# PKU-EPIC/HOTrack

Hardware: AMD Instinct MI355X
Metric: HandTrackNet point-cloud frames/sec (N=1024) (higher is better)
Workload: dtype f32; 1 GPU; HandTrackNet forward, batch=64 synthetic 1024-pt clouds per GPU (BASELINE configs[1]); per_gpu_batch=64, global_batch=64, npoints=1024, parallelism=dp1 (independent batches, no collective), world_size=1, resident_batches_rotated=5, dead_attention_elided=True, fused_sa_kernels=True, launch=hipGraph replay, batches_in_flight=4, hip_hw_queues=4, sa_compute_units=256, weights=deterministic random init (no checkpoint available offline)

## Files before the change

hotrack_amd/csrc/capi.hip:

```cpp
#include <stdlib.h>

#include "pn2_common.h"
#include "../../include/pn2_ext.h"

namespace pn2 {
static thread_local int g_last_hip_error = 0;
void set_last_hip_error(int e) { g_last_hip_error = e; }

int fps_dispatch(int b, int n, int m, const float *xyz, float *temp, int *idx, hipStream_t st, int force_threads,
                 const int *skip_flags, int nflags, float *radii);
int fps_tie_check(int b, int n, int m, int m1, const float *xyz, const int *idx, const float *radii, int *flags, hipStream_t st);
bool fps_knn_supported(int n, int nq, int k);
bool ball_tie_supported(long b, long n, long m, long m2);
int ball_tie_dispatch(int b, int n, int m, float radius, int nsample, const float *xyz, int *idx, const int *picks, float *new_xyz_out,
                      float *new_xyz_copy, int copy_ld, int m2, const float *radii, int *flags, hipStream_t st, int *counts);
bool three_nn_interp_supported(long b, long n, long m, long c, long ldp, long ldo);
int three_nn_interp_dispatch(int b, int n, int m, int c, const float *unknown, const float *known, const float *points, int ldp,
                             float *out, int ldo, hipStream_t st);
int fps_knn_dispatch(int b, int n, int m, const float *xyz, int *idx, float *radii, int nq, int k, int k2, const float *query,
                     int *kidx, int *kidx2, hipStream_t st);
int ball_query_dispatch(int b, int n, int m, float radius, int nsample, const float *new_xyz, const float *xyz,
                        int *idx, hipStream_t st, const int *picks, float *new_xyz_out, float *new_xyz_copy, int copy_ld, int *counts);
int three_nn_dispatch(int b, int n, int m, const float *unknown, const float *known, float *dist2, int *idx,
                      hipStream_t st, bool weights);
int interp_pm_dispatch(int b, int c, int m, int n, const float *points, int ldp, const int *idx, const float *weight,
                       float *out, int ldo, hipStream_t st);
int knn_dispatch(int b, int n, int m, int k, const float *unknown, const float *known, float *dist2, int *idx,
                 hipStream_t st, int k2, int *idx2);
int group_fwd_dispatch(int b, int c, int n, int npoints, int nsample, const float *points, const int *idx,
                       float *out, hipStream_t st);
int group_bwd_dispatch(int b, int c, int n, int npoints, int nsample, const float *grad_out, const int *idx,
                       float *grad_points, hipStream_t st);
int interp_fwd_dispatch(int b, int c, int m, int n, const float *points, const int *idx, const float *weight,
                        float *out, hipStream_t st);
int interp_bwd_dispatch(int b, int c, int n, int m, const float *grad_out, const int *idx, const float *weight,
                        float *grad_points, hipStream_t st);
}

using namespace pn2;

#define PN2_REQ(cond, code) \
// ... 206 lines not shown

int pn2x_three_nn_weights(int b, int n, int m, const float *unknown, const float *known, float *weight, int *idx,
                          void *stream) {
    PN2_REQ(b >= 0 && n >= 0 && m >= 3, PN2_EINVAL);
    if (b == 0 || n == 0) return PN2_OK;
    PN2_REQ(unknown && known && weight && idx, PN2_ENULL);
    PN2_REQ(b <= 65535 && fits_int((long)n * 3) && fits_int((long)m * 3), PN2_ERANGE);
    return three_nn_dispatch(b, n, m, unknown, known, weight, idx, (hipStream_t)stream, true);
}

int pn2x_three_nn_interpolate_pm_supported(int b, int n, int m, int c, int ldp, int ldo) {
    return three_nn_interp_supported(b, n, m, c, ldp, ldo) ? 1 : 0;
}

int pn2x_three_nn_interpolate_pm(int b, int n, int m, int c, const float *unknown, const float *known, const float *points, int ldp,
                                 float *out, int ldo, void *stream) {
    PN2_REQ(b >= 0 && n >= 0 && m >= 3 && c >= 1 && ldp >= c && ldo >= c, PN2_EINVAL);
    if (b == 0 || n == 0) return PN2_OK;
    PN2_REQ(unknown && known && points && out, PN2_ENULL);
    PN2_REQ(b <= 65535 && fits_int((long)n * 3) && fits_int((long)m * 3), PN2_ERANGE);
    return three_nn_interp_dispatch(b, n, m, c, unknown, known, points, ldp, out, ldo, (hipStream_t)stream);
}

int pn2x_three_interpolate_pm(int b, int c, int m, int n, const float *points, int ldp, const int *idx,
                              const float *weight, float *out, int ldo, void *stream) {
    PN2_REQ(b >= 0 && c >= 0 && m >= 1 && n >= 0 && ldp >= c && ldo >= c, PN2_EINVAL);
    if (b == 0 || c == 0 || n == 0) return PN2_OK;
    PN2_REQ(points && idx && weight && out, PN2_ENULL);
    PN2_REQ(fits_int((long)n * 3), PN2_ERANGE);
    return interp_pm_dispatch(b, c, m, n, points, ldp, idx, weight, out, ldo, (hipStream_t)stream);
}

}
```

hotrack_amd/csrc/nn_search.hip:

```cpp
#include "pn2_common.h"
#include "knn_wave.h"

namespace pn2 {

constexpr int kNnTile = 2048;

template <int THREADS, bool WEIGHTS>
__global__ void __launch_bounds__(THREADS)
three_nn_kernel(int n, int m, const float *__restrict__ unknown_all, const float *__restrict__ known_all,
                float *__restrict__ dist2_all, int *__restrict__ idx_all) {
    extern __shared__ __attribute__((aligned(16))) float4 sk[];
    const int b = blockIdx.y;
    const float *__restrict__ known = known_all + (size_t)b * m * 3;
    const int q = blockIdx.x * THREADS + threadIdx.x;
    const bool active = q < n;
    const float *__restrict__ u = unknown_all + ((size_t)b * n + (active ? q : 0)) * 3;
    const float ux = u[0], uy = u[1], uz = u[2];

    float b1 = __builtin_inff(), b2 = __builtin_inff(), b3 = __builtin_inff();
    int i1 = 0, i2 = 0, i3 = 0;

    for (int t0 = 0; t0 < m; t0 += kNnTile) {
        const int tn = (m - t0) < kNnTile ? (m - t0) : kNnTile;
        if (t0 > 0) __syncthreads();
// ... 70 lines not shown
    if (c > 0) {
        sd[c - 1][0][ql] = b1; sd[c - 1][1][ql] = b2; sd[c - 1][2][ql] = b3;
        si[c - 1][0][ql] = i1; si[c - 1][1][ql] = i2; si[c - 1][2][ql] = i3;
    }
    __syncthreads();
    if (c != 0 || !active) return;
#pragma unroll
    for (int cc = 0; cc < 3; ++cc)
#pragma unroll
        for (int e = 0; e < 3; ++e) insert(sd[cc][e][ql], si[cc][e][ql]);
    float *od = dist2_all + ((size_t)b * n + q) * 3;
    int *oi = idx_all + ((size_t)b * n + q) * 3;
    if constexpr (WEIGHTS) {
        const float r1 = 1.0f / (__builtin_sqrtf(b1) + 1e-8f), r2 = 1.0f / (__builtin_sqrtf(b2) + 1e-8f),
                    r3 = 1.0f / (__builtin_sqrtf(b3) + 1e-8f);
        const float norm = (r1 + r2) + r3;
        od[0] = r1 / norm; od[1] = r2 / norm; od[2] = r3 / norm;
    } else {
        od[0] = b1; od[1] = b2; od[2] = b3;
    }
    oi[0] = i1; oi[1] = i2; oi[2] = i3;
}

__global__ void __launch_bounds__(256)
three_nn_interp_kernel(int n, int m, int c4, const float *__restrict__ unknown_all, const float *__restrict__ known_all,
                       const float *__restrict__ points_all, int ldp, float *__restrict__ out_all, int ldo) {
    extern __shared__ __attribute__((aligned(16))) float4 sk[];
    __shared__ float sd[3][3][64];
    __shared__ int si[3][3][64];
    __shared__ float fw[3][64];
    __shared__ int fi[3][64];
    const int b = blockIdx.y;
    const float *__restrict__ known = known_all + (size_t)b * m * 3;
    const int ql = threadIdx.x & 63, c = threadIdx.x >> 6;
    const int q = blockIdx.x * 64 + ql;
    const bool active = q < n;
    const float *__restrict__ u = unknown_all + ((size_t)b * n + (active ? q : 0)) * 3;
    const float ux = u[0], uy = u[1], uz = u[2];
    for (int p = threadIdx.x; p < m; p += 256) {
        const float *src = known + (size_t)3 * p;
        sk[p] = make_float4(src[0], src[1], src[2], 0.f);
    }
    __syncthreads();
    float b1 = __builtin_inff(), b2 = __builtin_inff(), b3 = __builtin_inff();
    int i1 = 0, i2 = 0, i3 = 0;
    auto insert = [&](float d, int k) {
        const bool lt1 = d < b1, lt2 = d < b2, lt3 = d < b3;
        b3 = lt2 ? b2 : (lt3 ? d : b3);
        i3 = lt2 ? i2 : (lt3 ? k : i3);
        b2 = lt1 ? b1 : (lt2 ? d : b2);
        i2 = lt1 ? i1 : (lt2 ? k : i2);
        b1 = lt1 ? d : b1;
        i1 = lt1 ? k : i1;
    };
    const int len = (m + 3) / 4, p0 = c * len, p1 = min(m, p0 + len);
#pragma unroll 4
    for (int p = p0; p < p1; ++p) {
        const float4 kp = sk[p];
        insert(sqdist(ux, uy, uz, kp.x, kp.y, kp.z), p);
    }
    if (c > 0) {
        sd[c - 1][0][ql] = b1; sd[c - 1][1][ql] = b2; sd[c - 1][2][ql] = b3;
        si[c - 1][0][ql] = i1; si[c - 1][1][ql] = i2; si[c - 1][2][ql] = i3;
    }
    __syncthreads();
    if (c == 0) {
#pragma unroll
        for (int cc = 0; cc < 3; ++cc)
#pragma unroll
            for (int e = 0; e < 3; ++e) insert(sd[cc][e][ql], si[cc][e][ql]);
        const float r1 = 1.0f / (__builtin_sqrtf(b1) + 1e-8f), r2 = 1.0f / (__builtin_sqrtf(b2) + 1e-8f),
                    r3 = 1.0f / (__builtin_sqrtf(b3) + 1e-8f);
        const float norm = (r1 + r2) + r3;
        fw[0][ql] = r1 / norm; fw[1][ql] = r2 / norm; fw[2][ql] = r3 / norm;
        fi[0][ql] = i1; fi[1][ql] = i2; fi[2][ql] = i3;
    }
    __syncthreads();
    const int rows = min(64, n - (int)blockIdx.x * 64);
    const float *__restrict__ src = points_all + (size_t)b * m * ldp;
    float *__restrict__ dst = out_all + ((size_t)b * n + (size_t)blockIdx.x * 64) * ldo;
    for (int e = threadIdx.x; e < rows * c4; e += 256) {
        const int r = e / c4, col = e - r * c4;
        const float w0 = fw[0][r], w1 = fw[1][r], w2 = fw[2][r];
        const float4 a0 = *reinterpret_cast<const float4 *>(src + (size_t)fi[0][r] * ldp + 4 * col);
        const float4 a1 = *reinterpret_cast<const float4 *>(src + (size_t)fi[1][r] * ldp + 4 * col);
        const float4 a2 = *reinterpret_cast<const float4 *>(src + (size_t)fi[2][r] * ldp + 4 * col);
        float4 o;
        o.x = __builtin_fmaf(w2, a2.x, __builtin_fmaf(w0, a0.x, w1 * a1.x));
        o.y = __builtin_fmaf(w2, a2.y, __builtin_fmaf(w0, a0.y, w1 * a1.y));
        o.z = __builtin_fmaf(w2, a2.z, __builtin_fmaf(w0, a0.z, w1 * a1.z));
        o.w = __builtin_fmaf(w2, a2.w, __builtin_fmaf(w0, a0.w, w1 * a1.w));
        *reinterpret_cast<float4 *>(dst + (size_t)r * ldo + 4 * col) = o;
    }
}

bool three_nn_interp_supported(long b, long n, long m, long c, long ldp, long ldo) {
    return b * n >= 16384 && b * n < 256L * 1024 && m >= 16 && m <= kNnTile && c >= 4 && c % 4 == 0 && ldp % 4 == 0 && ldo % 4 == 0;
}

int three_nn_interp_dispatch(int b, int n, int m, int c, const float *unknown, const float *known, const float *points, int ldp,
                             float *out, int ldo, hipStream_t st) {
    if (b == 0 || n == 0) return PN2_OK;
    if (!three_nn_interp_supported(b, n, m, c, ldp, ldo) || (((uintptr_t)points | (uintptr_t)out) % 16) != 0) return PN2_ERANGE;
    dim3 grid((n + 63) / 64, b);
    hipLaunchKernelGGL(three_nn_interp_kernel, grid, dim3(256), (size_t)m * sizeof(float4), st, n, m, c / 4, unknown, known, points, ldp, out, ldo);
    return check_launch();
}

int three_nn_dispatch(int b, int n, int m, const float *unknown, const float *known, float *dist2,
                      int *idx, hipStream_t st, bool weights) {
    if (b == 0 || n == 0) return PN2_OK;
    if ((long)b * n < 256L * 1024 && m >= 16 && m <= kNnTile) {
        dim3 grid((n + 63) / 64, b);
        const size_t lds_split = (size_t)m * sizeof(float4);
        if (weights) hipLaunchKernelGGL((three_nn_split_kernel<true>), grid, dim3(256), lds_split, st, n, m, unknown, known, dist2, idx);
        else hipLaunchKernelGGL((three_nn_split_kernel<false>), grid, dim3(256), lds_split, st, n, m, unknown, known, dist2, idx);
        return check_launch();
    }
    const int tile_cap = m < kNnTile ? m : kNnTile;
    const size_t lds = (size_t)(tile_cap > 0 ? tile_cap : 1) * sizeof(float4);
    if ((long)b * n < 256L * 1024) {
        dim3 grid((n + 63) / 64, b);
        if (weights) hipLaunchKernelGGL((three_nn_kernel<64, true>), grid, dim3(64), lds, st, n, m, unknown, known, dist2, idx);
        else hipLaunchKernelGGL((three_nn_kernel<64, false>), grid, dim3(64), lds, st, n, m, unknown, known, dist2, idx);
    } else {
        dim3 grid((n + 255) / 256, b);
        if (weights) hipLaunchKernelGGL((three_nn_kernel<256, true>), grid, dim3(256), lds, st, n, m, unknown, known, dist2, idx);
        else hipLaunchKernelGGL((three_nn_kernel<256, false>), grid, dim3(256), lds, st, n, m, unknown, known, dist2, idx);
// ... 91 lines not shown
```

hotrack_amd/csrc/sa_fused.hip:

```cpp
#include <stdlib.h>

#include "pn2_common.h"
#include "../../include/pn2_ext.h"

#ifndef SA_PAD
#define SA_PAD 4
#endif

#ifndef SA_DEFER_EPILOGUE
#define SA_DEFER_EPILOGUE 0
#endif
#ifndef SA_OVERLAP_WRITEOUT
#define SA_OVERLAP_WRITEOUT 1
#endif
#ifndef SA_SCALAR_L1
#define SA_SCALAR_L1 0
#endif
#ifndef SA_LOADER_PRIO
#define SA_LOADER_PRIO 0
#endif
#ifndef SA_PROBE
#define SA_PROBE 0
#endif
#ifndef SA_PREFETCH
// ... 815 lines not shown
    switch (a.K) {
        case 16: return launch_sa_k<C1, C2, C3, WC, RTC, MINW, NB1, 16>(b, a, st);
        case 32: return launch_sa_k<C1, C2, C3, WC, RTC, MINW, NB1, 32>(b, a, st);
        case 64: return launch_sa_k<C1, C2, C3, WC, RTC, MINW, NB1, 64>(b, a, st);
    }
    return PN2_ERANGE;
}

#ifndef SA_RTC128
#define SA_RTC128 2
#endif
#ifndef SA_NB1
#define SA_NB1 2
#endif
static long long *g_sa_trace = nullptr;
static bool sa_ranges_ok(long b, long n, long s, long k, long a1f_ld, long cadd_ld, long c3, long out_s, long out_c) {
    const long lim = 0xffffffffL;
    if (out_s < 0 || out_c < 0 || 4 * ((s - 1) * out_s + (c3 - 1) * out_c + 1) >= lim) return false;
    return n < (1L << 24) && s < (1L << 24) && 4 * a1f_ld < (1L << 24) && 4 * cadd_ld < (1L << 24) &&
           4 * b * n * (a1f_ld > 3 ? a1f_ld : 3) <= lim && 4 * s * (cadd_ld > 3 ? cadd_ld : 3) <= lim && 4 * s * k <= lim;
}

constexpr int kClsThreads = 1024;
__global__ __launch_bounds__(kClsThreads) void sa_class_lists_kernel(int M, int S, int N, const int *__restrict__ counts,
                                                                      int *__restrict__ list, int *__restrict__ sizes) {
    __shared__ int scan[3][kClsThreads];
    const int tid = (int)threadIdx.x;
    const int per = (M + kClsThreads - 1) / kClsThreads;
    const long lo = (long)tid * per;
    const int i0 = (int)(lo < M ? lo : M), i1 = i0 + per < M ? i0 + per : M;
    int c0 = 0, c1 = 0, c2 = 0;
    for (int i = i0; i < i1; ++i) {
        const int k = counts[i];
        c0 += k > 16 ? 1 : 0;
        c1 += (k > 8 && k <= 16) ? 1 : 0;
        c2 += k <= 8 ? 1 : 0;
    }
    int s0 = c0, s1 = c1, s2 = c2;
    for (int d = 1; d < kClsThreads; d <<= 1) {
        scan[0][tid] = s0; scan[1][tid] = s1; scan[2][tid] = s2;
        __syncthreads();
        if (tid >= d) { s0 += scan[0][tid - d]; s1 += scan[1][tid - d]; s2 += scan[2][tid - d]; }
        __syncthreads();
    }
    scan[0][tid] = s0; scan[1][tid] = s1; scan[2][tid] = s2;
    __syncthreads();
    const int t0 = scan[0][kClsThreads - 1], t1 = scan[1][kClsThreads - 1], t2 = scan[2][kClsThreads - 1];
    int p0 = s0 - c0, p1 = t0 + s1 - c1, p2 = t0 + t1 + s2 - c2;
    int b = i0 / S, s = i0 - b * S;
    int4 *__restrict__ dst = reinterpret_cast<int4 *>(list);
    for (int i = i0; i < i1; ++i) {
        const int k = counts[i];
        const int4 rec = make_int4(i, b * N, b, s);
        if (k > 16) dst[p0++] = rec;
        else if (k > 8) dst[p1++] = rec;
        else dst[p2++] = rec;
        if (++s == S) { s = 0; ++b; }
    }
    if (tid == 0) { sizes[0] = t0; sizes[1] = t1; sizes[2] = t2; }
}
}

extern "C" int pn2x_sa_class_lists(int b, int s, int n, const int *counts, int *list, int *sizes, void *stream) {
    using namespace pn2;
    if (b < 0 || s < 1 || n < 1) return PN2_EINVAL;
    if ((long)b * s >= (1L << 24) || (long)b * n >= (1L << 24)) return PN2_ERANGE;
    if (!sizes) return PN2_ENULL;
    if (b > 0 && (!counts || !list)) return PN2_ENULL;
    if ((uintptr_t)list % 16 != 0) return PN2_EINVAL;
    hipLaunchKernelGGL(sa_class_lists_kernel, dim3(1), dim3(kClsThreads), 0, (hipStream_t)stream, b * s, s, n, counts, list, sizes);
    return check_launch();
}

extern "C" int pn2x_sa_mlp_max_classes_supported(int k, int c1, int c2, int c3) {
    return (k == 32 && ((c1 == 32 && c2 == 32 && c3 == 64) || (c1 == 64 && c2 == 64 && c3 == 128))) ? 1 : 0;
}

extern "C" int pn2x_sa_mlp_max_classes(int b, int n, int s, int k, int c1, int c2, int c3, const float *a1f, int a1f_ld,
                                       const float *xyz, const float *cxyz, const float *wx, const float *b1, const float *cadd,
                                       int cadd_ld, const int *idx, const int *cls_list, const int *cls_sizes,
                                       const float *w2, const float *b2, const float *w3, const float *b3, float *out,
                                       long out_b, int out_s, int out_c, void *stream) {
    using namespace pn2;
    if (b < 0 || n < 1 || s < 0 || k < 1) return PN2_EINVAL;
    if (b == 0 || s == 0) return PN2_OK;
    if (!idx || !cls_list || !cls_sizes || !w2 || !b2 || !w3 || !b3 || !out) return PN2_ENULL;
    if (!a1f && !xyz) return PN2_ENULL;
    if (xyz && (!cxyz || !wx)) return PN2_ENULL;
    if ((a1f && (a1f_ld < c1 || a1f_ld % 4)) || (cadd && (cadd_ld < c1 || cadd_ld % 4))) return PN2_EINVAL;
    if (!pn2x_sa_mlp_max_classes_supported(k, c1, c2, c3)) return PN2_ERANGE;
    if (!sa_ranges_ok(b, n, s, k, a1f ? a1f_ld : 0, cadd ? cadd_ld : 0, c3, out_s, out_c)) return PN2_ERANGE;
    const long lim = 0xffffffffL;
    if (out_b < 0 || (long)b * n >= (1L << 24) || (long)b * s >= (1L << 24) || 128L * b * s > lim ||
        4L * b * s * (cadd && cadd_ld > 3 ? cadd_ld : 3) > lim || 4 * ((b - 1) * out_b + (s - 1L) * out_s + (c3 - 1L) * out_c + 1) >= lim)
// ... 118 lines not shown
```

hotrack_amd/ext.py:

```python
from __future__ import annotations

import ctypes
import os

import torch

from . import pointnet2_hip as _native

_lib = _native._lib
_vp, _ci = ctypes.c_void_p, ctypes.c_int
_lib.pn2x_kabsch.argtypes = [_ci, _ci, _ci, _vp, _vp, _vp, _vp, _vp]
_lib.pn2x_kabsch.restype = _ci


def kabsch(x: torch.Tensor, y: torch.Tensor):
    x = x.float().contiguous()
    y = y.float().contiguous()
    if x.dim() == 2:
        x = x.unsqueeze(0)
    B, num, _ = y.shape
    xb = x.shape[0]
    if xb not in (1, B) or x.shape[1] != num:
        raise ValueError(f"kabsch: x {tuple(x.shape)} does not match y {tuple(y.shape)}")
    px = _native._ptr(x, "x", torch.float32, xb * num * 3)
# ... 59 lines not shown
    return bool(_lib.pn2x_sa_mlp_max_supported(k, c1, c2, c3))


def _rows(t: torch.Tensor, name: str, cols: int):
    if not t.is_cuda or t.dtype != torch.float32 or t.dim() != 3:
        raise TypeError(f"{name}: expected a 3-D float32 GPU tensor")
    B, R, C = t.shape
    if C < cols or t.stride(2) != 1 or (R > 1 and B > 1 and t.stride(0) != R * t.stride(1)):
        raise ValueError(f"{name}: unsupported layout shape={tuple(t.shape)} strides={t.stride()}")
    return t.data_ptr(), t.stride(1)


def sa_mlp_max(idx: torch.Tensor, w2, b2, w3, b3, *, a1f=None, xyz=None, cxyz=None, wx=None, b1=None, cadd=None,
               out=None, point_major=False) -> torch.Tensor:
    return _sa_mlp_max(idx, w2, b2, w3, b3, None, a1f, xyz, cxyz, wx, b1, cadd, out, point_major)


_lib.pn2x_sa_mlp_max_classes.argtypes = [_ci] * 7 + [_vp, _ci, _vp, _vp, _vp, _vp, _vp, _ci, _vp, _vp, _vp, _vp, _vp, _vp, _vp, _vp, _cl, _ci, _ci, _vp]
_lib.pn2x_sa_mlp_max_classes.restype = _ci
_lib.pn2x_sa_mlp_max_classes_supported.argtypes = [_ci] * 4
_lib.pn2x_sa_mlp_max_classes_supported.restype = _ci
_lib.pn2x_sa_class_lists.argtypes = [_ci, _ci, _ci, _vp, _vp, _vp, _vp]
_lib.pn2x_sa_class_lists.restype = _ci


def sa_mlp_max_classes_supported(k: int, c1: int, c2: int, c3: int) -> bool:
    return bool(_lib.pn2x_sa_mlp_max_classes_supported(k, c1, c2, c3))


def sa_class_partition(counts: torch.Tensor):
    c = counts.reshape(-1)
    ids = torch.arange(c.numel(), dtype=torch.int32, device=c.device)
    masks = (c > 16, (c > 8) & (c <= 16), c <= 8)
    return torch.cat([ids[m] for m in masks]), torch.stack([m.sum() for m in masks]).to(torch.int32)


def sa_class_lists(counts: torch.Tensor, n: int):
    if not isinstance(counts, torch.Tensor) or counts.dim() != 2 or counts.dtype != torch.int32 or not counts.is_cuda:
        raise TypeError("sa_class_lists: counts must be a (B,S) int32 GPU tensor")
    if int(n) < 1:
        raise ValueError("sa_class_lists: n >= 1")
    B, S = counts.shape
    pc = _native._ptr(counts, "counts", torch.int32, B * S)
    lst = torch.empty((B * S, 4), dtype=torch.int32, device=counts.device)
    sizes = torch.empty(3, dtype=torch.int32, device=counts.device)
    with torch.cuda.device(counts.device):
        _native._check(_native._call(_lib.pn2x_sa_class_lists, "sa_class_lists_kernel", None, B, S, int(n), pc, lst.data_ptr(),
                                     sizes.data_ptr(), _native._stream(counts)), "sa_class_lists")
    return lst, sizes


def sa_mlp_max_classes(idx: torch.Tensor, classes, w2, b2, w3, b3, *, a1f=None, xyz=None, cxyz=None, wx=None, b1=None, cadd=None,
                       out=None, point_major=False) -> torch.Tensor:
    if not (isinstance(classes, (tuple, list)) and len(classes) == 2):
        raise TypeError("sa_mlp_max_classes: classes must be the (list, sizes) pair of sa_class_lists")
    return _sa_mlp_max(idx, w2, b2, w3, b3, classes, a1f, xyz, cxyz, wx, b1, cadd, out, point_major)


def _sa_mlp_max(idx, w2, b2, w3, b3, classes, a1f, xyz, cxyz, wx, b1, cadd, out, point_major):
    B, S, K = idx.shape
    C1, C2, C3 = w2.shape[1], w2.shape[0], w3.shape[0]
    f32 = torch.float32
    N = a1f.shape[1] if a1f is not None else xyz.shape[1]
    pa, lda = (None, 0) if a1f is None else _rows(a1f, "a1f", C1)
    pc, ldc = (None, 0) if cadd is None else _rows(cadd, "cadd", C1)
    px = None if xyz is None else _native._ptr(xyz, "xyz", f32, B * N * 3)
    pcx = None if cxyz is None else _native._ptr(cxyz, "cxyz", f32, B * S * 3)
    pwx = None if wx is None else _native._ptr(wx, "wx", f32, C1 * 3)
    pb1 = None if b1 is None else _native._ptr(b1, "b1", f32, C1)
    pi = _native._ptr(idx, "idx", torch.int32, B * S * K)
    pw2, pb2 = _native._ptr(w2, "w2", f32, C2 * C1), _native._ptr(b2, "b2", f32, C2)
    pw3, pb3 = _native._ptr(w3, "w3", f32, C3 * C2), _native._ptr(b3, "b3", f32, C3)
# ... 120 lines not shown
    with torch.cuda.device(unknown.device):
        _native._check(_lib.pn2x_three_nn_weights(B, n, m, _native._ptr(unknown, "unknown", f32, B * n * 3),
                                                  _native._ptr(known, "known", f32, B * m * 3), w.data_ptr(), idx.data_ptr(),
                                                  _native._stream(unknown)), "three_nn_weights")
    return w, idx


def three_interpolate_pm(points: torch.Tensor, idx: torch.Tensor, weight: torch.Tensor, out: torch.Tensor) -> torch.Tensor:
    B, M, C = points.shape
    n = idx.shape[1]
    pp, ldp = _rows(points, "points", C)
    po, ldo = _rows(out, "out", C)
    with torch.cuda.device(points.device):
        _native._check(_lib.pn2x_three_interpolate_pm(B, C, M, n, pp, ldp, _native._ptr(idx, "idx", torch.int32, B * n * 3),
                                                      _native._ptr(weight, "weight", torch.float32, B * n * 3), po, ldo,
                                                      _native._stream(points)), "three_interpolate_pm")
    return out


_lib.pn2x_three_nn_interpolate_pm.argtypes = [_ci, _ci, _ci, _ci, _vp, _vp, _vp, _ci, _vp, _ci, _vp]
_lib.pn2x_three_nn_interpolate_pm.restype = _ci
_lib.pn2x_three_nn_interpolate_pm_supported.argtypes = [_ci] * 6
_lib.pn2x_three_nn_interpolate_pm_supported.restype = _ci


def three_nn_interpolate_pm(unknown: torch.Tensor, known: torch.Tensor, points: torch.Tensor, out: torch.Tensor) -> torch.Tensor:
    B, n, _ = unknown.shape
    m, C = known.shape[1], points.shape[2]
    pp, ldp = _rows(points, "points", C)
    po, ldo = _rows(out, "out", C)
    f32 = torch.float32
    if _lib.pn2x_three_nn_interpolate_pm_supported(B, n, m, C, ldp, ldo) and pp % 16 == 0 and po % 16 == 0:
        with torch.cuda.device(points.device):
            _native._check(_native._call(_lib.pn2x_three_nn_interpolate_pm, "three_nn_interp_kernel", None, B, n, m, C,
                                         _native._ptr(unknown, "unknown", f32, B * n * 3), _native._ptr(known, "known", f32, B * m * 3),
                                         pp, ldp, po, ldo, _native._stream(points)), "three_nn_interpolate_pm")
        return out
    w, i3 = three_nn_weights(unknown, known)
    return three_interpolate_pm(points, i3, w, out)


def gather_rows(src: torch.Tensor, idx: torch.Tensor) -> torch.Tensor:
    B, N, C = src.shape
    M = idx.shape[1]
    out = torch.empty((B, M, C), dtype=torch.float32, device=src.device)
    with torch.cuda.device(src.device):
        _native._check(_lib.pn2x_gather_rows(B, N, M, C, _native._ptr(src, "src", torch.float32, B * N * C),
                                             _native._ptr(idx, "idx", torch.int32, B * M), out.data_ptr(),
                                             _native._stream(src)), "gather_rows")
    return out


def bias_act_pm_(y: torch.Tensor, bias: torch.Tensor, rows_per_bias: int, relu: bool = True) -> torch.Tensor:
    B, R, C = y.shape
# ... 845 lines not shown
```

include/pn2_ext.h:

```cpp
#ifndef PN2_EXT_H
#define PN2_EXT_H

#include "pn2_hip.h"

#ifdef __cplusplus
extern "C" {
#endif

int pn2x_kabsch(int b, int xb, int num, const float *x, const float *y, float *R, float *t, void *stream);
int pn2x_kabsch_backward(int b, int xb, int num, const float *x, const float *y, const float *R, const float *grad_R,
                         const float *grad_t, float *grad_y, void *stream);

int pn2x_hand_frame(int b, int xb, int num, int n, int j, const float *palm_template, const float *kp,
                    const int *palm_idx, const float *points, float scale, float *R, float *t, float *xyz2,
                    float *xyz1, float *xyz2_copy, int copy_ld, int *nonfinite, void *stream);

int pn2x_sa_mlp_max(int b, int n, int s, int k, int c1, int c2, int c3, const float *a1f, int a1f_ld,
                    const float *xyz, const float *cxyz, const float *wx, const float *b1, const float *cadd,
                    int cadd_ld, const int *idx,
                    const float *w2, const float *b2, const float *w3, const float *b3, float *out,
                    long out_b, int out_s, int out_c, void *stream);
int pn2x_sa_mlp_max_supported(int k, int c1, int c2, int c3);

int pn2x_sa_class_lists(int b, int s, int n, const int *counts, int *list, int *sizes, void *stream);
int pn2x_sa_mlp_max_classes_supported(int k, int c1, int c2, int c3);
int pn2x_sa_mlp_max_classes(int b, int n, int s, int k, int c1, int c2, int c3, const float *a1f, int a1f_ld,
                            const float *xyz, const float *cxyz, const float *wx, const float *b1, const float *cadd,
                            int cadd_ld, const int *idx, const int *cls_list, const int *cls_sizes,
                            const float *w2, const float *b2, const float *w3, const float *b3, float *out,
                            long out_b, int out_s, int out_c, void *stream);

int pn2x_bias_act(int b, int c, int n, float *y, const float *bias, int relu, void *stream);

int pn2x_three_nn_weights(int b, int n, int m, const float *unknown, const float *known, float *weight, int *idx,
                          void *stream);

int pn2x_three_nn_interpolate_pm_supported(int b, int n, int m, int c, int ldp, int ldo);
int pn2x_three_nn_interpolate_pm(int b, int n, int m, int c, const float *unknown, const float *known, const float *points, int ldp,
                                 float *out, int ldo, void *stream);
int pn2x_three_interpolate_pm(int b, int c, int m, int n, const float *points, int ldp, const int *idx,
                              const float *weight, float *out, int ldo, void *stream);

int pn2x_furthest_point_sampling_radii(int b, int n, int m, const float *xyz, int *idx, float *radii, void *stream);
int pn2x_fps_radii_knn_supported(int n, int nq, int k);
int pn2x_fps_radii_knn(int b, int n, int m, const float *xyz, int *idx, float *radii, int nq, int k, int k2, const float *query,
                       int *knn_idx, int *knn_idx2, void *stream);
int pn2x_fps_prefix_ties(int b, int n, int m1, int m2, const float *xyz, const int *idx1, const float *radii, int *flags, void *stream);
int pn2x_ball_query_picks_ties_supported(int b, int n, int m, int m2);
int pn2x_ball_query_picks_ties(int b, int n, int m, float radius, int nsample, const float *xyz, const int *picks, float *new_xyz,
                               int *idx, float *new_xyz_copy, int copy_ld, int m2, const float *radii, int *flags, void *stream);
int pn2x_fps_prefix_flags(int n);
int pn2x_furthest_point_sampling_prefix(int b, int n, int m, const float *xyz, const int *flags, int nflags, int *idx, void *stream);

int pn2x_knn_indices(int b, int n, int m, int k, int k2, const float *unknown, const float *known, int *idx, int *idx2, void *stream);

int pn2x_ball_query_picks(int b, int n, int m, float radius, int nsample, const float *xyz, const int *picks, float *new_xyz,
                          int *idx, float *new_xyz_copy, int copy_ld, void *stream);
int pn2x_ball_query_picks_counts(int b, int n, int m, float radius, int nsample, const float *xyz, const int *picks, float *new_xyz,
                                 int *idx, float *new_xyz_copy, int copy_ld, int *counts, void *stream);
int pn2x_ball_query_picks_ties_counts(int b, int n, int m, float radius, int nsample, const float *xyz, const int *picks, float *new_xyz,
                                      int *idx, float *new_xyz_copy, int copy_ld, int m2, const float *radii, int *flags, int *counts,
                                      void *stream);

long pn2x_ball_query_grid_scratch_words(int b, int n);
// ... 289 lines not shown
```

network/models/fast_eval.py:

```python
from __future__ import annotations

import torch
import torch.nn.functional as F



def _lin_relu(x2d: torch.Tensor, W: torch.Tensor, b: torch.Tensor) -> torch.Tensor:
    from hotrack_amd import ext
    return ext.linear(x2d, W, b, relu=True)


def _lin(x2d: torch.Tensor, W: torch.Tensor, b: torch.Tensor = None) -> torch.Tensor:
    from hotrack_amd import ext
    return ext.linear(x2d, W, b)


class FastEval:
    MAX_POINTS = 16384

    def __init__(self, net):
        self.net = net
        self._shapes_seen = set()
        self._key = None
        self.P = None
# ... 206 lines not shown
        if classes:
            _, l1_xyz, i_l2, idx1, cnt1, knn_lists = ext.fps_two_level(xyz2, S1, bh.sa2.npoint, query=(bh.sa1.radius_list[0], K1),
                                                                       knn=knn_req, query_counts=True)
        else:
            _, l1_xyz, i_l2, idx1, knn_lists = ext.fps_two_level(xyz2, S1, bh.sa2.npoint, query=(bh.sa1.radius_list[0], K1), knn=knn_req)
        return dict(cnt1=cnt1, P=P, pts=pts, B=B, N=N, J=J, c_i=c_i, fp1_in=fp1_in, nonfinite=nonfinite, R=R, t=t, xyz2=xyz2, xyz1=xyz1,
                    canon=canon, S1=S1, K1=K1, l1_xyz=l1_xyz, i_l2=i_l2, idx1=idx1, knn_lists=knn_lists)

    def _dense(self, G, flag_dict):
        from hotrack_amd import ext
        from hotrack_amd import pointnet2_utils as ops
        net, bh = self.net, self.net.bhand
        P, pts, B, N, J, c_i, fp1_in, nonfinite = G["P"], G["pts"], G["B"], G["N"], G["J"], G["c_i"], G["fp1_in"], G["nonfinite"]
        R, t, xyz2, xyz1, canon, S1, K1 = G["R"], G["t"], G["xyz2"], G["xyz1"], G["canon"], G["S1"], G["K1"]
        l1_xyz, i_l2, idx1, knn_lists = G["l1_xyz"], G["i_l2"], G["idx1"], G["knn_lists"]
        f32 = dict(dtype=torch.float32, device=pts.device)
        dev = net.device
        p = P["sa1"]
        c_l1 = p["l3"][0].shape[0]
        fp2_w = P["fp2"][0][0].shape[1]
        fp2_in = torch.empty((B, S1, fp2_w), **f32)
        l1_feat = fp2_in[:, :, :c_l1]
        cnt1 = G["cnt1"]
        if cnt1 is not None:
            ext.sa_mlp_max_classes(idx1, ext.sa_class_lists(cnt1, N), *p["l2"], *p["l3"], xyz=xyz2, cxyz=l1_xyz, wx=p["wx"], b1=p["b1"],
                                   out=l1_feat)
        else:
            ext.sa_mlp_max(idx1, *p["l2"], *p["l3"], xyz=xyz2, cxyz=l1_xyz, wx=p["wx"], b1=p["b1"], out=l1_feat)

        p = P["sa2"]
        S2, K2 = bh.sa2.npoint, bh.sa2.nsample_list[0]
        c_l2 = p["l3"][0].shape[0]
        sa3_in = torch.empty((B, S2, c_l2 + 4), **f32)
        if cnt1 is not None:
            idx2, l2_xyz, cnt2 = ext.ball_query_picks(bh.sa2.radius_list[0], K2, l1_xyz, i_l2, xyz_copy=sa3_in[:, :, c_l2:c_l2 + 3], counts=True)
        else:
            idx2, l2_xyz = ext.ball_query_picks(bh.sa2.radius_list[0], K2, l1_xyz, i_l2, xyz_copy=sa3_in[:, :, c_l2:c_l2 + 3])
        a1f = _lin(l1_feat.reshape(B * S1, c_l1), p["w1f"]).view(B, S1, -1)
        l2_feat = sa3_in[:, :, :c_l2]
        if cnt1 is not None:
            ext.sa_mlp_max_classes(idx2, ext.sa_class_lists(cnt2, S1), *p["l2"], *p["l3"], a1f=a1f, xyz=l1_xyz, cxyz=l2_xyz, wx=p["wx"],
                                   b1=p["b1"], out=l2_feat)
        else:
            ext.sa_mlp_max(idx2, *p["l2"], *p["l3"], a1f=a1f, xyz=l1_xyz, cxyz=l2_xyz, wx=p["wx"], b1=p["b1"], out=l2_feat)

        large = self._large_batch(B, N)
        mc = P["mid_chain"]
        if large and mc is not None:
            part = ext.sa3_chain(sa3_in, *mc["sa3"])
            l2_out = ext.fp3_chain(sa3_in, part, mc["wgt"], mc["bg"], mc["wa"], mc["wf"], mc["bf"])
        else:
            x = sa3_in.view(B * S2, c_l2 + 4)[:, :c_l2 + 3]
            for W, b in P["sa3"]:
                x = _lin_relu(x, W, b)
            l3 = ext.max_rows(x.view(B, S2, -1))

            p = P["fp3"]
            g = _lin(l3, p["wb"], p["b"])
            if B == 1:
                h = _lin_relu(sa3_in.view(S2, c_l2 + 4)[:, :c_l2], p["wa"], g.view(-1)).view(B, S2, -1)
            else:
                h = _lin(sa3_in.view(B * S2, c_l2 + 4)[:, :c_l2], p["wa"]).view(B, S2, -1)
                ext.bias_act_pm_(h, g, rows_per_bias=S2, relu=True)
            x = h.view(B * S2, -1)
            for W, b in p["rest"]:
                x = _lin_relu(x, W, b)
            l2_out = x.view(B, S2, -1)

        ext.three_nn_interpolate_pm(l1_xyz, l2_xyz, l2_out, fp2_in[:, :, c_l1:])
        x = fp2_in.view(B * S1, fp2_w)
        for W, b in P["fp2"]:
            x = _lin_relu(x, W, b)
        l1_out = x.view(B, S1, -1)

        assert c_i == l1_out.shape[2]
        ext.three_nn_interpolate_pm(xyz2, l1_xyz, l1_out, fp1_in[:, :, :c_i])
        q = P["q"]
        Ks = [q[("q1", i)]["K"] for i in range(2)]
        kmin, kmax = min(Ks), max(Ks)
        gi, gi_small = knn_lists
        c_q = q[("q1", 0)]["l3"][0].shape[0]
        c1q = q[("q1", 0)]["l2"][0].shape[1]
        rc = P["row_chain"]
        if large and rc is not None and gi_small is not None:
            lst, counts = ext.row_lists(gi, gi_small, N)
            a_all = torch.empty((B, N, 4 * c1q), **f32)
            ext.row_chain(fp1_in, lst, counts, rc["wa"], rc["ba"], rc["wb"], rc["bb"], rc["wc"], rc["bc"], rc["wq"], out=a_all)
        else:
            f = P["fp1_fused"]
            if f is not None:
                x = ext.mlp2_rows(fp1_in.view(B * N, c_i + 4), f["w2"], f["b2"], f["w3"], f["b3"], w2e=f["w2e"])
            else:
                x = fp1_in.view(B * N, c_i + 4)[:, :c_i + 3]
                for W, b in P["fp1"]:
                    x = _lin_relu(x, W, b)
            src2 = _lin_relu(x, *P["conv1"])
            a_all = _lin(src2, P["wq"]).view(B, N, -1)
        plan = []
        for i, K in enumerate(Ks):
            j = P["wq_order"].index(i)
            idx = gi if K == kmax else (gi_small if K == kmin and gi_small is not None else gi[:, :, :K].contiguous())
            plan.append((idx, a_all[:, :, 2 * c1q * j:2 * c1q * (j + 1)], xyz2))
        f11 = torch.empty((B, J, 2 * c_q), **f32)
        self._q_scales(ext, "q1", plan, q, xyz1, c1q, 0, None, f11, c_q)
        Wr, br, perm = P["r1"]
        f12 = _lin(ext.gather_rows(f11, self._perm_idx(perm, B)).view(B * J, -1), Wr, br)
        cadd = _lin(f12, P["wc2"]).view(B, J, -1)
        f13 = torch.empty((B, J, 2 * c_q), **f32)
        self._q_scales(ext, "q2", plan, q, xyz1, c1q, c1q, cadd, f13, c_q)
        Wr, br, perm = P["r2"]
        f14 = _lin(ext.gather_rows(f13, self._perm_idx(perm, B)).view(B * J, -1), Wr, br)
# ... 30 lines not shown
```

Measured before the change: 90960 frames/s.

## Interpolate only kNN-referenced rows and batch both SA class-list builds

The final three-NN interpolation into fp1_in now runs only for the rows named in the row_lists output (the rows the downstream row_chain actually reads), instead of all N points per batch. The two SA class-list kernels are merged into one launch that handles both problems in separate blocks. That kernel is also rewritten to use 2-bit class codes, popcount tallies and a wave-shuffle scan instead of a 1024-step shared-memory scan. This cuts interpolation work and kernel launches, at the cost of leaving the unreferenced rows of fp1_in unwritten and adding scattered row writes.

```diff
diff --git a/hotrack_amd/csrc/capi.hip b/hotrack_amd/csrc/capi.hip
--- a/hotrack_amd/csrc/capi.hip
+++ b/hotrack_amd/csrc/capi.hip
@@ -17,6 +17,9 @@
 bool three_nn_interp_supported(long b, long n, long m, long c, long ldp, long ldo);
 int three_nn_interp_dispatch(int b, int n, int m, int c, const float *unknown, const float *known, const float *points, int ldp,
                              float *out, int ldo, hipStream_t st);
+bool three_nn_interp_rows_supported(long b, long n, long m, long c, long ldp, long ldo);
+int three_nn_interp_rows_dispatch(int b, int n, int m, int c, const float *unknown, const float *known, const float *points, int ldp,
+                                  float *out, int ldo, const int *row_list, const int *row_counts, hipStream_t st);
 int fps_knn_dispatch(int b, int n, int m, const float *xyz, int *idx, float *radii, int nq, int k, int k2, const float *query,
                      int *kidx, int *kidx2, hipStream_t st);
 int ball_query_dispatch(int b, int n, int m, float radius, int nsample, const float *new_xyz, const float *xyz,
@@ -269,6 +272,19 @@
     return three_nn_interp_dispatch(b, n, m, c, unknown, known, points, ldp, out, ldo, (hipStream_t)stream);
 }
 
+int pn2x_three_nn_interpolate_pm_rows_supported(int b, int n, int m, int c, int ldp, int ldo) {
+    return three_nn_interp_rows_supported(b, n, m, c, ldp, ldo) ? 1 : 0;
+}
+
+int pn2x_three_nn_interpolate_pm_rows(int b, int n, int m, int c, const float *unknown, const float *known, const float *points,
+                                      int ldp, float *out, int ldo, const int *row_list, const int *row_counts, void *stream) {
+    PN2_REQ(b >= 0 && n >= 0 && m >= 3 && c >= 1 && ldp >= c && ldo >= c, PN2_EINVAL);
+    if (b == 0 || n == 0) return PN2_OK;
+    PN2_REQ(unknown && known && points && out && row_list && row_counts, PN2_ENULL);
+    PN2_REQ(b <= 65535 && fits_int((long)n * 3) && fits_int((long)m * 3), PN2_ERANGE);
+    return three_nn_interp_rows_dispatch(b, n, m, c, unknown, known, points, ldp, out, ldo, row_list, row_counts, (hipStream_t)stream);
+}
+
 int pn2x_three_interpolate_pm(int b, int c, int m, int n, const float *points, int ldp, const int *idx,
                               const float *weight, float *out, int ldo, void *stream) {
     PN2_REQ(b >= 0 && c >= 0 && m >= 1 && n >= 0 && ldp >= c && ldo >= c, PN2_EINVAL);
diff --git a/hotrack_amd/csrc/nn_search.hip b/hotrack_amd/csrc/nn_search.hip
--- a/hotrack_amd/csrc/nn_search.hip
+++ b/hotrack_amd/csrc/nn_search.hip
@@ -116,19 +116,29 @@
     oi[0] = i1; oi[1] = i2; oi[2] = i3;
 }
 
+template <bool ROWS>
 __global__ void __launch_bounds__(256)
 three_nn_interp_kernel(int n, int m, int c4, const float *__restrict__ unknown_all, const float *__restrict__ known_all,
-                       const float *__restrict__ points_all, int ldp, float *__restrict__ out_all, int ldo) {
+                       const float *__restrict__ points_all, int ldp, float *__restrict__ out_all, int ldo,
+                       const int *__restrict__ row_list, const int *__restrict__ row_counts) {
     extern __shared__ __attribute__((aligned(16))) float4 sk[];
     __shared__ float sd[3][3][64];
     __shared__ int si[3][3][64];
     __shared__ float fw[3][64];
     __shared__ int fi[3][64];
+    __shared__ int fq[ROWS ? 64 : 1];
     const int b = blockIdx.y;
     const float *__restrict__ known = known_all + (size_t)b * m * 3;
     const int ql = threadIdx.x & 63, c = threadIdx.x >> 6;
-    const int q = blockIdx.x * 64 + ql;
-    const bool active = q < n;
+    int q = blockIdx.x * 64 + ql, nq = n;
+    if constexpr (ROWS) {
+        nq = row_counts[2 * b + 1];
+        nq = nq < 0 ? 0 : (nq > n ? n : nq);
+        if ((int)blockIdx.x * 64 >= nq) return;
+        q = q < nq ? row_list[(size_t)b * n + q] : -1;
+        if ((unsigned)q >= (unsigned)n) q = -1;
+    }
+    const bool active = ROWS ? q >= 0 : q < n;
     const float *__restrict__ u = unknown_all + ((size_t)b * n + (active ? q : 0)) * 3;
     const float ux = u[0], uy = u[1], uz = u[2];
     for (int p = threadIdx.x; p < m; p += 256) {
@@ -168,11 +178,12 @@
         const float norm = (r1 + r2) + r3;
         fw[0][ql] = r1 / norm; fw[1][ql] = r2 / norm; fw[2][ql] = r3 / norm;
         fi[0][ql] = i1; fi[1][ql] = i2; fi[2][ql] = i3;
-    }
-    __syncthreads();
-    const int rows = min(64, n - (int)blockIdx.x * 64);
+        if constexpr (ROWS) fq[ql] = q;
+    }
+    __syncthreads();
+    const int rows = min(64, nq - (int)blockIdx.x * 64);
     const float *__restrict__ src = points_all + (size_t)b * m * ldp;
-    float *__restrict__ dst = out_all + ((size_t)b * n + (size_t)blockIdx.x * 64) * ldo;
+    float *__restrict__ dst = out_all + ((size_t)b * n + (ROWS ? (size_t)0 : (size_t)blockIdx.x * 64)) * ldo;
     for (int e = threadIdx.x; e < rows * c4; e += 256) {
         const int r = e / c4, col = e - r * c4;
         const float w0 = fw[0][r], w1 = fw[1][r], w2 = fw[2][r];
@@ -184,7 +195,11 @@
         o.y = __builtin_fmaf(w2, a2.y, __builtin_fmaf(w0, a0.y, w1 * a1.y));
         o.z = __builtin_fmaf(w2, a2.z, __builtin_fmaf(w0, a0.z, w1 * a1.z));
         o.w = __builtin_fmaf(w2, a2.w, __builtin_fmaf(w0, a0.w, w1 * a1.w));
-        *reinterpret_cast<float4 *>(dst + (size_t)r * ldo + 4 * col) = o;
+        if constexpr (ROWS) {
+            if (fq[r] >= 0) *reinterpret_cast<float4 *>(dst + (size_t)fq[r] * ldo + 4 * col) = o;
+        } else {
+            *reinterpret_cast<float4 *>(dst + (size_t)r * ldo + 4 * col) = o;
+        }
     }
 }
 
@@ -197,7 +212,22 @@
     if (b == 0 || n == 0) return PN2_OK;
     if (!three_nn_interp_supported(b, n, m, c, ldp, ldo) || (((uintptr_t)points | (uintptr_t)out) % 16) != 0) return PN2_ERANGE;
     dim3 grid((n + 63) / 64, b);
-    hipLaunchKernelGGL(three_nn_interp_kernel, grid, dim3(256), (size_t)m * sizeof(float4), st, n, m, c / 4, unknown, known, points, ldp, out, ldo);
+    hipLaunchKernelGGL(three_nn_interp_kernel<false>, grid, dim3(256), (size_t)m * sizeof(float4), st, n, m, c / 4, unknown, known, points,
+                       ldp, out, ldo, nullptr, nullptr);
+    return check_launch();
+}
+
+bool three_nn_interp_rows_supported(long b, long n, long m, long c, long ldp, long ldo) {
+    return b <= 65535 && m >= 3 && m <= kNnTile && c >= 4 && c % 4 == 0 && ldp % 4 == 0 && ldo % 4 == 0;
+}
+
+int three_nn_interp_rows_dispatch(int b, int n, int m, int c, const float *unknown, const float *known, const float *points, int ldp,
+                                  float *out, int ldo, const int *row_list, const int *row_counts, hipStream_t st) {
+    if (b == 0 || n == 0) return PN2_OK;
+    if (!three_nn_interp_rows_supported(b, n, m, c, ldp, ldo) || (((uintptr_t)points | (uintptr_t)out) % 16) != 0) return PN2_ERANGE;
+    dim3 grid((n + 63) / 64, b);
+    hipLaunchKernelGGL(three_nn_interp_kernel<true>, grid, dim3(256), (size_t)m * sizeof(float4), st, n, m, c / 4, unknown, known, points,
+                       ldp, out, ldo, row_list, row_counts);
     return check_launch();
 }
 
diff --git a/hotrack_amd/csrc/sa_fused.hip b/hotrack_amd/csrc/sa_fused.hip
--- a/hotrack_amd/csrc/sa_fused.hip
+++ b/hotrack_amd/csrc/sa_fused.hip
@@ -861,54 +861,127 @@
 }
 
 constexpr int kClsThreads = 1024;
-__global__ __launch_bounds__(kClsThreads) void sa_class_lists_kernel(int M, int S, int N, const int *__restrict__ counts,
-                                                                      int *__restrict__ list, int *__restrict__ sizes) {
-    __shared__ int scan[3][kClsThreads];
-    const int tid = (int)threadIdx.x;
-    const int per = (M + kClsThreads - 1) / kClsThreads;
-    const long lo = (long)tid * per;
-    const int i0 = (int)(lo < M ? lo : M), i1 = i0 + per < M ? i0 + per : M;
+constexpr int kClsCached = 32;
+struct ClsProblem {
+    int M, S, N;
+    const int *counts;
+    int *list, *sizes;
+};
+
+__device__ __forceinline__ unsigned cls_code(int k) { return k > 16 ? 0u : (k > 8 ? 1u : 2u); }
+
+__device__ __forceinline__ unsigned cls_load4(const int *__restrict__ counts, int i, int M, bool vec) {
+    if (i >= M) return 0xffu;
+    if (vec && i + 3 < M) {
+        const int4 v = *reinterpret_cast<const int4 *>(counts + i);
+        return cls_code(v.x) | (cls_code(v.y) << 2) | (cls_code(v.z) << 4) | (cls_code(v.w) << 6);
+    }
+    unsigned c = 0xffu;
+#pragma unroll
+    for (int u = 0; u < 4; ++u)
+        if (i + u < M) c = (c & ~(3u << (2 * u))) | (cls_code(counts[i + u]) << (2 * u));
+    return c;
+}
+
+template <bool CACHE>
+__global__ __launch_bounds__(kClsThreads) void sa_class_lists2_kernel(ClsProblem q0, ClsProblem q1) {
+    __shared__ int wave_tot[3][kClsThreads / 64];
+    const ClsProblem P = blockIdx.x == 0 ? q0 : q1;
+    const int M = P.M, S = P.S, N = P.N;
+    const int tid = (int)threadIdx.x, lane = tid & 63, wave = tid >> 6;
+    const int per = ((M + kClsThreads - 1) / kClsThreads + 3) & ~3;
+    const int i0 = tid * per;
+    const bool vec = ((uintptr_t)P.counts & 15) == 0;
+    constexpr unsigned long long kEven = 0x5555555555555555ull;
+    unsigned long long codes = ~0ull;
     int c0 = 0, c1 = 0, c2 = 0;
-    for (int i = i0; i < i1; ++i) {
-        const int k = counts[i];
-        c0 += k > 16 ? 1 : 0;
-        c1 += (k > 8 && k <= 16) ? 1 : 0;
-        c2 += k <= 8 ? 1 : 0;
+    auto tally = [&](unsigned long long w) {
+        const unsigned long long lo = w & kEven, hi = (w >> 1) & kEven;
+        c0 += __builtin_popcountll(~lo & ~hi & kEven);
+        c1 += __builtin_popcountll(lo & ~hi);
+        c2 += __builtin_popcountll(~lo & hi);
+    };
+    if constexpr (CACHE) {
+        unsigned w[kClsCached / 4];
+#pragma unroll
+        for (int g = 0; g < kClsCached / 4; ++g) w[g] = 4 * g < per ? cls_load4(P.counts, i0 + 4 * g, M, vec) : 0xffu;
+        codes = 0ull;
+#pragma unroll
+        for (int g = 0; g < kClsCached / 4; ++g) codes |= (unsigned long long)w[g] << (8 * g);
+        tally(codes);
+    } else {
+        for (int g = 0; g < per; g += 4) tally(0xffffffffffffff00ull | cls_load4(P.counts, i0 + g, M, vec));
     }
     int s0 = c0, s1 = c1, s2 = c2;
-    for (int d = 1; d < kClsThreads; d <<= 1) {
-        scan[0][tid] = s0; scan[1][tid] = s1; scan[2][tid] = s2;
-        __syncthreads();
-        if (tid >= d) { s0 += scan[0][tid - d]; s1 += scan[1][tid - d]; s2 += scan[2][tid - d]; }
-        __syncthreads();
-    }
-    scan[0][tid] = s0; scan[1][tid] = s1; scan[2][tid] = s2;
+#pragma unroll
+    for (int d = 1; d < 64; d <<= 1) {
+        const int u0 = __shfl_up(s0, d), u1 = __shfl_up(s1, d), u2 = __shfl_up(s2, d);
+        if (lane >= d) { s0 += u0; s1 += u1; s2 += u2; }
+    }
+    if (lane == 63) { wave_tot[0][wave] = s0; wave_tot[1][wave] = s1; wave_tot[2][wave] = s2; }
     __syncthreads();
-    const int t0 = scan[0][kClsThreads - 1], t1 = scan[1][kClsThreads - 1], t2 = scan[2][kClsThreads - 1];
-    int p0 = s0 - c0, p1 = t0 + s1 - c1, p2 = t0 + t1 + s2 - c2;
+    int o0 = 0, o1 = 0, o2 = 0, t0 = 0, t1 = 0, t2 = 0;
+#pragma unroll
+    for (int w = 0; w < kClsThreads / 64; ++w) {
+        const int v0 = wave_tot[0][w], v1 = wave_tot[1][w], v2 = wave_tot[2][w];
+        t0 += v0; t1 += v1; t2 += v2;
+        if (w < wave) { o0 += v0; o1 += v1; o2 += v2; }
+    }
+    if (tid == 0) { P.sizes[0] = t0; P.sizes[1] = t1; P.sizes[2] = t2; }
+    if (i0 >= M) return;
+    int p0 = o0 + s0 - c0, p1 = t0 + o1 + s1 - c1, p2 = t0 + t1 + o2 + s2 - c2;
     int b = i0 / S, s = i0 - b * S;
-    int4 *__restrict__ dst = reinterpret_cast<int4 *>(list);
-    for (int i = i0; i < i1; ++i) {
-        const int k = counts[i];
-        const int4 rec = make_int4(i, b * N, b, s);
-        if (k > 16) dst[p0++] = rec;
-        else if (k > 8) dst[p1++] = rec;
-        else dst[p2++] = rec;
+    int4 *__restrict__ dst = reinterpret_cast<int4 *>(P.list);
+    auto place = [&](int i, unsigned code) {
+        if (code == 3u) return;
+        const int pos = code == 0u ? p0 : (code == 1u ? p1 : p2);
+        p0 += code == 0u; p1 += code == 1u; p2 += code == 2u;
+        if (pos < M) dst[pos] = make_int4(i, b * N, b, s);
         if (++s == S) { s = 0; ++b; }
-    }
-    if (tid == 0) { sizes[0] = t0; sizes[1] = t1; sizes[2] = t2; }
-}
-}
-
-extern "C" int pn2x_sa_class_lists(int b, int s, int n, const int *counts, int *list, int *sizes, void *stream) {
-    using namespace pn2;
+    };
+    if constexpr (CACHE) {
+#pragma unroll
+        for (int j = 0; j < kClsCached; ++j) place(i0 + j, (unsigned)(codes >> (2 * j)) & 3u);
+    } else {
+        for (int g = 0; g < per; g += 4) {
+            const unsigned w = cls_load4(P.counts, i0 + g, M, vec);
+#pragma unroll
+            for (int u = 0; u < 4; ++u) place(i0 + g + u, (w >> (2 * u)) & 3u);
+        }
+    }
+}
+
+static int cls_check(int b, int s, int n, const int *counts, const int *list, const int *sizes) {
     if (b < 0 || s < 1 || n < 1) return PN2_EINVAL;
     if ((long)b * s >= (1L << 24) || (long)b * n >= (1L << 24)) return PN2_ERANGE;
     if (!sizes) return PN2_ENULL;
     if (b > 0 && (!counts || !list)) return PN2_ENULL;
     if ((uintptr_t)list % 16 != 0) return PN2_EINVAL;
-    hipLaunchKernelGGL(sa_class_lists_kernel, dim3(1), dim3(kClsThreads), 0, (hipStream_t)stream, b * s, s, n, counts, list, sizes);
+    return PN2_OK;
+}
+
+static int launch_class_lists(int problems, const ClsProblem &q0, const ClsProblem &q1, hipStream_t st) {
+    const int m = q0.M > q1.M ? q0.M : q1.M;
+    if (m <= kClsThreads * kClsCached) hipLaunchKernelGGL(sa_class_lists2_kernel<true>, dim3(problems), dim3(kClsThreads), 0, st, q0, q1);
+    else hipLaunchKernelGGL(sa_class_lists2_kernel<false>, dim3(problems), dim3(kClsThreads), 0, st, q0, q1);
     return check_launch();
+}
+}
+
+extern "C" int pn2x_sa_class_lists(int b, int s, int n, const int *counts, int *list, int *sizes, void *stream) {
+    using namespace pn2;
+    if (const int rc = cls_check(b, s, n, counts, list, sizes); rc != PN2_OK) return rc;
+    const ClsProblem q = {b * s, s, n, counts, list, sizes};
+    return launch_class_lists(1, q, q, (hipStream_t)stream);
+}
+
+extern "C" int pn2x_sa_class_lists2(int b0, int s0, int n0, const int *counts0, int *list0, int *sizes0, int b1, int s1, int n1,
+                                    const int *counts1, int *list1, int *sizes1, void *stream) {
+    using namespace pn2;
+    if (const int rc = cls_check(b0, s0, n0, counts0, list0, sizes0); rc != PN2_OK) return rc;
+    if (const int rc = cls_check(b1, s1, n1, counts1, list1, sizes1); rc != PN2_OK) return rc;
+    const ClsProblem q0 = {b0 * s0, s0, n0, counts0, list0, sizes0}, q1 = {b1 * s1, s1, n1, counts1, list1, sizes1};
+    return launch_class_lists(2, q0, q1, (hipStream_t)stream);
 }
 
 extern "C" int pn2x_sa_mlp_max_classes_supported(int k, int c1, int c2, int c3) {
diff --git a/hotrack_amd/ext.py b/hotrack_amd/ext.py
--- a/hotrack_amd/ext.py
+++ b/hotrack_amd/ext.py
@@ -105,6 +105,8 @@
 _lib.pn2x_sa_mlp_max_classes_supported.restype = _ci
 _lib.pn2x_sa_class_lists.argtypes = [_ci, _ci, _ci, _vp, _vp, _vp, _vp]
 _lib.pn2x_sa_class_lists.restype = _ci
+_lib.pn2x_sa_class_lists2.argtypes = [_ci, _ci, _ci, _vp, _vp, _vp] * 2 + [_vp]
+_lib.pn2x_sa_class_lists2.restype = _ci
 
 
 def sa_mlp_max_classes_supported(k: int, c1: int, c2: int, c3: int) -> bool:
@@ -118,19 +120,35 @@
     return torch.cat([ids[m] for m in masks]), torch.stack([m.sum() for m in masks]).to(torch.int32)
 
 
-def sa_class_lists(counts: torch.Tensor, n: int):
+def _class_lists_args(counts, n, what):
     if not isinstance(counts, torch.Tensor) or counts.dim() != 2 or counts.dtype != torch.int32 or not counts.is_cuda:
-        raise TypeError("sa_class_lists: counts must be a (B,S) int32 GPU tensor")
+        raise TypeError(f"{what}: counts must be a (B,S) int32 GPU tensor")
     if int(n) < 1:
-        raise ValueError("sa_class_lists: n >= 1")
+        raise ValueError(f"{what}: n >= 1")
     B, S = counts.shape
     pc = _native._ptr(counts, "counts", torch.int32, B * S)
     lst = torch.empty((B * S, 4), dtype=torch.int32, device=counts.device)
     sizes = torch.empty(3, dtype=torch.int32, device=counts.device)
+    return B, S, int(n), pc, lst, sizes
+
+
+def sa_class_lists(counts: torch.Tensor, n: int):
+    B, S, n, pc, lst, sizes = _class_lists_args(counts, n, "sa_class_lists")
     with torch.cuda.device(counts.device):
-        _native._check(_native._call(_lib.pn2x_sa_class_lists, "sa_class_lists_kernel", None, B, S, int(n), pc, lst.data_ptr(),
+        _native._check(_native._call(_lib.pn2x_sa_class_lists, "sa_class_lists2_kernel", None, B, S, n, pc, lst.data_ptr(),
                                      sizes.data_ptr(), _native._stream(counts)), "sa_class_lists")
     return lst, sizes
+
+
+def sa_class_lists_pair(counts_a: torch.Tensor, n_a: int, counts_b: torch.Tensor, n_b: int):
+    a = _class_lists_args(counts_a, n_a, "sa_class_lists_pair")
+    b = _class_lists_args(counts_b, n_b, "sa_class_lists_pair")
+    if counts_a.device != counts_b.device:
+        raise ValueError("sa_class_lists_pair: both problems on one device")
+    with torch.cuda.device(counts_a.device):
+        _native._check(_native._call(_lib.pn2x_sa_class_lists2, "sa_class_lists2_kernel", None, *a[:4], a[4].data_ptr(), a[5].data_ptr(),
+                                     *b[:4], b[4].data_ptr(), b[5].data_ptr(), _native._stream(counts_a)), "sa_class_lists_pair")
+    return (a[4], a[5]), (b[4], b[5])
 
 
 def sa_mlp_max_classes(idx: torch.Tensor, classes, w2, b2, w3, b3, *, a1f=None, xyz=None, cxyz=None, wx=None, b1=None, cadd=None,
@@ -297,14 +315,38 @@
 _lib.pn2x_three_nn_interpolate_pm.restype = _ci
 _lib.pn2x_three_nn_interpolate_pm_supported.argtypes = [_ci] * 6
 _lib.pn2x_three_nn_interpolate_pm_supported.restype = _ci
-
-
-def three_nn_interpolate_pm(unknown: torch.Tensor, known: torch.Tensor, points: torch.Tensor, out: torch.Tensor) -> torch.Tensor:
+_lib.pn2x_three_nn_interpolate_pm_rows.argtypes = [_ci, _ci, _ci, _ci, _vp, _vp, _vp, _ci, _vp, _ci, _vp, _vp, _vp]
+_lib.pn2x_three_nn_interpolate_pm_rows.restype = _ci
+_lib.pn2x_three_nn_interpolate_pm_rows_supported.argtypes = [_ci] * 6
+_lib.pn2x_three_nn_interpolate_pm_rows_supported.restype = _ci
+
+
+def three_nn_interpolate_pm(unknown: torch.Tensor, known: torch.Tensor, points: torch.Tensor, out: torch.Tensor, rows=None) -> torch.Tensor:
+    if rows is not None:
+        if not (isinstance(rows, (tuple, list)) and len(rows) == 2 and all(isinstance(t, torch.Tensor) for t in rows)):
+            raise TypeError("three_nn_interpolate_pm: rows must be the (list, counts) pair of row_lists")
+        if rows[0].dtype != torch.int32 or rows[1].dtype != torch.int32:
+            raise TypeError("three_nn_interpolate_pm: rows must be int32 tensors")
+        if tuple(rows[0].shape) != tuple(unknown.shape[:2]) or tuple(rows[1].shape) != (unknown.shape[0], 2):
+            raise ValueError("three_nn_interpolate_pm: rows must be list (B,n) and counts (B,2)")
     B, n, _ = unknown.shape
     m, C = known.shape[1], points.shape[2]
     pp, ldp = _rows(points, "points", C)
     po, ldo = _rows(out, "out", C)
     f32 = torch.float32
+    if rows is not None:
+        if not (_lib.pn2x_three_nn_interpolate_pm_rows_supported(B, n, m, C, ldp, ldo) and pp % 16 == 0 and po % 16 == 0):
+            raise ValueError("three_nn_interpolate_pm: rows needs 3 <= m <= 2048 known points, C and the row strides multiples of 4 "
+                             "and 16-byte aligned points / out")
+        if rows[0].device != points.device or rows[1].device != points.device:
+            raise ValueError("three_nn_interpolate_pm: rows on another device than points")
+        with torch.cuda.device(points.device):
+            _native._check(_native._call(_lib.pn2x_three_nn_interpolate_pm_rows, "three_nn_interp_kernel", None, B, n, m, C,
+                                         _native._ptr(unknown, "unknown", f32, B * n * 3), _native._ptr(known, "known", f32, B * m * 3),
+                                         pp, ldp, po, ldo, _native._ptr(rows[0], "rows list", torch.int32, B * n),
+                                         _native._ptr(rows[1], "rows counts", torch.int32, B * 2), _native._stream(points)),
+                           "three_nn_interpolate_pm")
+        return out
     if _lib.pn2x_three_nn_interpolate_pm_supported(B, n, m, C, ldp, ldo) and pp % 16 == 0 and po % 16 == 0:
         with torch.cuda.device(points.device):
             _native._check(_native._call(_lib.pn2x_three_nn_interpolate_pm, "three_nn_interp_kernel", None, B, n, m, C,
diff --git a/include/pn2_ext.h b/include/pn2_ext.h
--- a/include/pn2_ext.h
+++ b/include/pn2_ext.h
@@ -23,6 +23,8 @@
 int pn2x_sa_mlp_max_supported(int k, int c1, int c2, int c3);
 
 int pn2x_sa_class_lists(int b, int s, int n, const int *counts, int *list, int *sizes, void *stream);
+int pn2x_sa_class_lists2(int b0, int s0, int n0, const int *counts0, int *list0, int *sizes0, int b1, int s1, int n1,
+                         const int *counts1, int *list1, int *sizes1, void *stream);
 int pn2x_sa_mlp_max_classes_supported(int k, int c1, int c2, int c3);
 int pn2x_sa_mlp_max_classes(int b, int n, int s, int k, int c1, int c2, int c3, const float *a1f, int a1f_ld,
                             const float *xyz, const float *cxyz, const float *wx, const float *b1, const float *cadd,
@@ -40,6 +42,9 @@
                                  float *out, int ldo, void *stream);
 int pn2x_three_interpolate_pm(int b, int c, int m, int n, const float *points, int ldp, const int *idx,
                               const float *weight, float *out, int ldo, void *stream);
+int pn2x_three_nn_interpolate_pm_rows_supported(int b, int n, int m, int c, int ldp, int ldo);
+int pn2x_three_nn_interpolate_pm_rows(int b, int n, int m, int c, const float *unknown, const float *known, const float *points,
+                                      int ldp, float *out, int ldo, const int *row_list, const int *row_counts, void *stream);
 
 int pn2x_furthest_point_sampling_radii(int b, int n, int m, const float *xyz, int *idx, float *radii, void *stream);
 int pn2x_fps_radii_knn_supported(int n, int nq, int k);
diff --git a/network/models/fast_eval.py b/network/models/fast_eval.py
--- a/network/models/fast_eval.py
+++ b/network/models/fast_eval.py
@@ -252,25 +252,23 @@
         fp2_in = torch.empty((B, S1, fp2_w), **f32)
         l1_feat = fp2_in[:, :, :c_l1]
         cnt1 = G["cnt1"]
-        if cnt1 is not None:
-            ext.sa_mlp_max_classes(idx1, ext.sa_class_lists(cnt1, N), *p["l2"], *p["l3"], xyz=xyz2, cxyz=l1_xyz, wx=p["wx"], b1=p["b1"],
-                                   out=l1_feat)
-        else:
-            ext.sa_mlp_max(idx1, *p["l2"], *p["l3"], xyz=xyz2, cxyz=l1_xyz, wx=p["wx"], b1=p["b1"], out=l1_feat)
-
-        p = P["sa2"]
+        p2 = P["sa2"]
         S2, K2 = bh.sa2.npoint, bh.sa2.nsample_list[0]
-        c_l2 = p["l3"][0].shape[0]
+        c_l2 = p2["l3"][0].shape[0]
         sa3_in = torch.empty((B, S2, c_l2 + 4), **f32)
         if cnt1 is not None:
             idx2, l2_xyz, cnt2 = ext.ball_query_picks(bh.sa2.radius_list[0], K2, l1_xyz, i_l2, xyz_copy=sa3_in[:, :, c_l2:c_l2 + 3], counts=True)
-        else:
+            cls1, cls2 = ext.sa_class_lists_pair(cnt1, N, cnt2, S1)
+            ext.sa_mlp_max_classes(idx1, cls1, *p["l2"], *p["l3"], xyz=xyz2, cxyz=l1_xyz, wx=p["wx"], b1=p["b1"], out=l1_feat)
+        else:
+            ext.sa_mlp_max(idx1, *p["l2"], *p["l3"], xyz=xyz2, cxyz=l1_xyz, wx=p["wx"], b1=p["b1"], out=l1_feat)
             idx2, l2_xyz = ext.ball_query_picks(bh.sa2.radius_list[0], K2, l1_xyz, i_l2, xyz_copy=sa3_in[:, :, c_l2:c_l2 + 3])
+
+        p = p2
         a1f = _lin(l1_feat.reshape(B * S1, c_l1), p["w1f"]).view(B, S1, -1)
         l2_feat = sa3_in[:, :, :c_l2]
         if cnt1 is not None:
-            ext.sa_mlp_max_classes(idx2, ext.sa_class_lists(cnt2, S1), *p["l2"], *p["l3"], a1f=a1f, xyz=l1_xyz, cxyz=l2_xyz, wx=p["wx"],
-                                   b1=p["b1"], out=l2_feat)
+            ext.sa_mlp_max_classes(idx2, cls2, *p["l2"], *p["l3"], a1f=a1f, xyz=l1_xyz, cxyz=l2_xyz, wx=p["wx"], b1=p["b1"], out=l2_feat)
         else:
             ext.sa_mlp_max(idx2, *p["l2"], *p["l3"], a1f=a1f, xyz=l1_xyz, cxyz=l2_xyz, wx=p["wx"], b1=p["b1"], out=l2_feat)
 
@@ -304,7 +302,6 @@
         l1_out = x.view(B, S1, -1)
 
         assert c_i == l1_out.shape[2]
-        ext.three_nn_interpolate_pm(xyz2, l1_xyz, l1_out, fp1_in[:, :, :c_i])
         q = P["q"]
         Ks = [q[("q1", i)]["K"] for i in range(2)]
         kmin, kmax = min(Ks), max(Ks)
@@ -314,9 +311,11 @@
         rc = P["row_chain"]
         if large and rc is not None and gi_small is not None:
             lst, counts = ext.row_lists(gi, gi_small, N)
+            ext.three_nn_interpolate_pm(xyz2, l1_xyz, l1_out, fp1_in[:, :, :c_i], rows=(lst, counts))
             a_all = torch.empty((B, N, 4 * c1q), **f32)
             ext.row_chain(fp1_in, lst, counts, rc["wa"], rc["ba"], rc["wb"], rc["bb"], rc["wc"], rc["bc"], rc["wq"], out=a_all)
         else:
+            ext.three_nn_interpolate_pm(xyz2, l1_xyz, l1_out, fp1_in[:, :, :c_i])
             f = P["fp1_fused"]
             if f is not None:
                 x = ext.mlp2_rows(fp1_in.view(B * N, c_i + 4), f["w2"], f["b2"], f["w3"], f["b3"], w2e=f["w2e"])
```

Measured after the change: 92500 frames/s, median of 6. +1.7%, better.
